# kch3782/torcwa

Measured on AMD Instinct MI355X. Metric: RCWA layer-solves/sec (complex64 I/O) at Fourier order [15,15], higher is better.
Workload: dtype c128 results (mixed-precision eigensolver: fp32 eigendecomposition refined to fp64 by two Newton steps -- fp64 residual and update GEMMs, the correction solved with ONE fp32 LU of the fp32 start; everything else fp64 MFMA); complex64 I/O; 1 GPU; configs[1]: single patterned layer, order=[15,15] (n=1922), 300x300 grid, 128-lambda sweep, glass input half-space; points_total=128, points_per_gpu=128, layer_solves_per_point=1, chunk=128, streams=1, precision=high

## Files before the change

torcwa_amd/csrc/eig.hip:

```cpp
#include "eig.hpp"
#include "prof.hpp"
#include <cstdlib>
#include <string>
#include <vector>

namespace trx {

static inline size_t al256(size_t x) { return (x + 255) & ~(size_t)255; }

static int eig_vec_env() {
    const char* e = getenv("TRX_EIG_VEC");
    const int v = e ? atoi(e) : 0;
    return (v == 0 || v == 1 || v == 3) ? v : 0;
}
static int g_eig_vec = eig_vec_env();
static thread_local int tl_eig_vec = -1, tl_refine = -1;
static thread_local int tl_last_fallback = 0;
static inline int cur_eig_vec() { return tl_eig_vec >= 0 ? tl_eig_vec : g_eig_vec; }
struct EigCallOpts {
    EigCallOpts(unsigned opts) { const int r = opts & 0xF, v = (opts >> 4) & 0xF; tl_refine = r ? r : -1; tl_eig_vec = v ? v : -1; }
    ~EigCallOpts() { tl_refine = -1; tl_eig_vec = -1; }
};
bool eig_uses_mixed(int n, int batch, size_t elem) { return elem == 8 && ((cur_eig_vec() == 3 && n >= 8) || (cur_eig_vec() == 0 && n >= 256 && batch >= 8)); }
int eig_set_knob(const char* key, int value) {
    if (std::string(key) != "eig_vec" || (value != 0 && value != 1 && value != 3)) return TRX_ERR_ARG;
    g_eig_vec = value;
    return TRX_OK;
}


template <class T> size_t eig_ws_bytes_t(int n, int batch);
static size_t eig_ws_bytes_f32(int n, int batch) { return eig_ws_bytes_t<float>(n, batch); }

static size_t mixed_pool_bytes(int n, int batch) {
    const size_t B = batch, N = n;
    return al256(8 * B * N * N) + al256(eig_ws_bytes_f32(n, batch)) + al256(8 * B * N * N) + al256(8 * B * N);
}
static size_t mixed_extra_bytes(int n, int batch) {
    const size_t B = batch, N = n, e = 16;
    const size_t zx = 2 * al256(e * B * N * N), pool = mixed_pool_bytes(n, batch);
    size_t tot = 0;
    if (pool > zx) tot += al256(pool - zx);
    tot += al256(sizeof(int) * B * N) * 3 + al256(sizeof(int) * (B + 2)) * 2 + al256(sizeof(int) * B) + al256(sizeof(int) * 2 * REFINE_EDGE_CAP * B) +
           al256(8 * B) * 2 + al256(8 * 64 * B) + al256(REFINE_CLUSTER_BYTES * B) + al256(e * B * N);
    return tot;
}

template <class T>
size_t eig_ws_bytes_t(int n, int batch) {
    const size_t e = sizeof(cx<T>), B = batch, N = n;
    size_t tot = 0;
    tot += al256(e * B * N * N) * 2;
    tot += al256(e * B * N * EigPlan::HNB) * 2;
    tot += al256(e * B * EigPlan::HNB * EigPlan::HNB);
    tot += al256(e * B * EigPlan::HNB * N) * 2;
    tot += al256(e * B * N * 2 * EigPlan::HNB) * 2;
    tot += al256(e * B * EigPlan::HNB * EigPlan::HNB);
    tot += al256(e * B * N * EigPlan::HGK) * 3 + al256(e * B * EigPlan::HGK * EigPlan::HGK) * 2;
    tot += al256(e * B * EigPlan::HNB) * 2;
    tot += al256(e * B * EigPlan::QW * EigPlan::QW);
    {
        const size_t slots = (size_t)qr_log_slots(n) * qr_chains_for(batch);
        tot += al256(e * B * slots * EigPlan::QW * EigPlan::QW) + al256(sizeof(QrLink) * B * slots);
    }
    tot += al256(e * B * EigPlan::QKC * EigPlan::QNS);
    tot += al256(sizeof(T) * B * N) + al256(sizeof(T) * 3 * B * N) + al256(sizeof(int) * 2 * B);
    tot += al256(sizeof(QrState) * B);
    tot += al256(sizeof(int) * 128 + sizeof(long long) * 24);
    if (eig_uses_mixed(n, batch, sizeof(T))) tot += mixed_extra_bytes(n, batch);
    return tot;
}

template <class T>
void eig_carve(EigBuffers<T>& Bf, void* A, void* ws, int n, int batch) {
    const size_t e = sizeof(cx<T>), B = batch, N = n;
    char* p = (char*)ws;
    auto take = [&](size_t bytes) { char* q = p; p += al256(bytes); return q; };
    Bf.A = (cx<T>*)A;
    Bf.Z = (cx<T>*)take(e * B * N * N);
    Bf.X = (cx<T>*)take(e * B * N * N);
    Bf.mixed_pool = nullptr;
    Bf.mixed_pool_bytes = 0;
    if (eig_uses_mixed(n, batch, sizeof(T))) {
        const size_t zx = 2 * al256(e * B * N * N), pool = mixed_pool_bytes(n, batch);
        if (pool > zx) (void)take(pool - zx);
        Bf.mixed_pool = (char*)Bf.Z;
        Bf.mixed_pool_bytes = pool > zx ? pool : zx;
    }
    Bf.Vp = (cx<T>*)take(e * B * N * EigPlan::HNB);
    Bf.Yp = (cx<T>*)take(e * B * N * EigPlan::HNB);
    Bf.Tp = (cx<T>*)take(e * B * EigPlan::HNB * EigPlan::HNB);
    Bf.W1 = (cx<T>*)take(e * B * EigPlan::HNB * N);
    Bf.W2 = (cx<T>*)take(e * B * EigPlan::HNB * N);
    Bf.YV = (cx<T>*)take(e * B * N * 2 * EigPlan::HNB);
    Bf.BC = (cx<T>*)take(e * B * N * 2 * EigPlan::HNB);
    Bf.Sm = (cx<T>*)take(e * B * EigPlan::HNB * EigPlan::HNB);
    Bf.Vg = (cx<T>*)take(e * B * N * EigPlan::HGK);
    Bf.Wg = (cx<T>*)take(e * B * N * EigPlan::HGK);
    Bf.W2g = (cx<T>*)take(e * B * N * EigPlan::HGK);
    Bf.Tg = (cx<T>*)take(e * B * EigPlan::HGK * EigPlan::HGK);
    Bf.Gg = (cx<T>*)take(e * B * EigPlan::HGK * EigPlan::HGK);
    Bf.tau = (cx<T>*)take(e * B * EigPlan::HNB);
    Bf.tvec = (cx<T>*)take(e * B * EigPlan::HNB);
    Bf.U = (cx<T>*)take(e * B * EigPlan::QW * EigPlan::QW);
    {
        const size_t slots = (size_t)qr_log_slots(n) * qr_chains_for(batch);
        Bf.Ulog = (cx<T>*)take(e * B * slots * EigPlan::QW * EigPlan::QW);
        Bf.links = (QrLink*)take(sizeof(QrLink) * B * slots);
    }
    Bf.shifts = (cx<T>*)take(e * B * EigPlan::QKC * EigPlan::QNS);
    Bf.bal_d = (T*)take(sizeof(T) * B * N);
    Bf.bal_w = (T*)take(sizeof(T) * 3 * B * N);
    Bf.bal_flags = (int*)take(sizeof(int) * 2 * B);
    Bf.st = (QrState*)take(sizeof(QrState) * B);
    Bf.summary = (int*)take(sizeof(int) * 128 + sizeof(long long) * 24);
    Bf.r_piv = Bf.r_linfo = Bf.r_flags = Bf.r_partner = Bf.r_clus = Bf.r_edges = Bf.r_ecount = nullptr;
    Bf.r_eoff = Bf.r_lmax = Bf.r_scan = nullptr;
    Bf.r_tab = nullptr;
    Bf.r_d0 = nullptr;
    if (eig_uses_mixed(n, batch, sizeof(T))) {
        Bf.r_piv = (int*)take(sizeof(int) * B * N);
        Bf.r_partner = (int*)take(sizeof(int) * B * N);
        Bf.r_clus = (int*)take(sizeof(int) * B * N);
        Bf.r_linfo = (int*)take(sizeof(int) * (B + 2));
        Bf.r_flags = (int*)take(sizeof(int) * (B + 2));
        Bf.r_ecount = (int*)take(sizeof(int) * B);
        Bf.r_edges = (int*)take(sizeof(int) * 2 * REFINE_EDGE_CAP * B);
        Bf.r_eoff = (T*)take(8 * B);
        Bf.r_lmax = (T*)take(8 * B);
        Bf.r_scan = (T*)take(8 * 64 * B);
        Bf.r_tab = take(REFINE_CLUSTER_BYTES * B);
        Bf.r_d0 = (cx<T>*)take(e * B * N);
    }
}

namespace {
__global__ __launch_bounds__(256) void cvt_c128_c64_kernel(const cx<double>* __restrict__ in, cx<float>* __restrict__ out, long count) {
    const long i = (long)blockIdx.x * blockDim.x + threadIdx.x;
    if (i < count) { const cx<double> v = in[i]; out[i] = cx<float>((float)v.x, (float)v.y); }
}
int eig_mixed_convert(hipStream_t s, const cx<double>* in, cx<float>* out, long count) {
    TRX_LAUNCH(cvt_c128_c64_kernel, dim3(cdiv_i(count, 256)), dim3(256), 0, s, in, out, count);
    TRX_CHECK_LAUNCH();
    return TRX_OK;
}

template <class T>
__global__ __launch_bounds__(256) void clear_below_subdiag_kernel(cx<T>* __restrict__ Aall, int n) {
    cx<T>* A = Aall + (long)blockIdx.z * n * n;
    const int j = blockIdx.x * blockDim.x + threadIdx.x;
    const int i = blockIdx.y;
    if (j < n && i > j + 1) A[(long)i * n + j] = cx<T>(T(0), T(0));
}

template <class T>
int eig_after_balance(hipStream_t s, const EigBuffers<T>& B, void* w, void* V, int n, int batch, int* info);

template <class T>
__global__ __launch_bounds__(256) void gather_rows_kernel(const T* __restrict__ src, T* __restrict__ dst, const int* __restrict__ idx, long row, int to_compact) {
    const long i = (long)blockIdx.x * blockDim.x + threadIdx.x;
    if (i >= row) return;
    const long j = blockIdx.y, b = idx[j];
    if (to_compact) dst[j * row + i] = src[b * row + i];
    else dst[b * row + i] = src[j * row + i];
}

template <class T>
int eig_redo_subset(hipStream_t s, void* A, void* w, void* V, int n, int batch, int* info, void* ws, size_t ws_bytes, const T* bal_d, const std::vector<int>& bad, int nf) {
    const size_t e = sizeof(cx<T>), N = n, NF = nf;
    struct RouteGuard { int save; RouteGuard() : save(tl_eig_vec) { tl_eig_vec = 1; } ~RouteGuard() { tl_eig_vec = save; } } guard;
    const size_t front = eig_ws_bytes_t<T>(n, nf);
    const size_t tail = al256(e * NF * N * N) * 2 + al256(e * NF * N) + al256(sizeof(T) * NF * N) + al256(sizeof(int) * NF) * 2;
    if (front + tail > ws_bytes) return TRX_ERR_WORKSPACE;
    char* p = (char*)ws + ws_bytes - tail;
    p = (char*)(((size_t)p) & ~(size_t)255);
    if (p < (char*)ws + front) return TRX_ERR_WORKSPACE;
    auto take = [&](size_t bytes) { char* q = p; p += al256(bytes); return q; };
    char* p_save = p;
    p = p_save + al256(e * NF * N * N) * 2;
    cx<T>* wsub = (cx<T>*)take(e * NF * N);
    T* dsub = (T*)take(sizeof(T) * NF * N);
    int* idx = (int*)take(sizeof(int) * NF);
    int* isub = (int*)take(sizeof(int) * NF);
    p = p_save;
    if ((const char*)wsub < (const char*)(bal_d + (size_t)batch * n)) return TRX_ERR_WORKSPACE;
    cx<T>* Asub = (cx<T>*)take(e * NF * N * N);
    cx<T>* Vsub = (cx<T>*)take(e * NF * N * N);
    std::vector<int> hidx;
    for (int b = 0; b < batch; ++b) if (bad[b]) hidx.push_back(b);
    if ((int)hidx.size() != nf) return TRX_ERR_ARG;
    if (hipMemcpyAsync(idx, hidx.data(), sizeof(int) * NF, hipMemcpyHostToDevice, s) != hipSuccess) return TRX_ERR_LAUNCH;
    if (hipStreamSynchronize(s) != hipSuccess) return TRX_ERR_LAUNCH;
    TRX_LAUNCH((gather_rows_kernel<T>), dim3(cdiv_i(n, 256), nf), dim3(256), 0, s, bal_d, dsub, (const int*)idx, (long)n, 1);
    TRX_LAUNCH((gather_rows_kernel<cx<T>>), dim3(cdiv_i((long)n * n, 256), nf), dim3(256), 0, s, (const cx<T>*)A, Asub, (const int*)idx, (long)n * n, 1);
    EigBuffers<T> S;
    eig_carve<T>(S, Asub, ws, n, nf);
    if (hipMemcpyAsync(S.bal_d, dsub, sizeof(T) * NF * N, hipMemcpyDeviceToDevice, s) != hipSuccess) return TRX_ERR_LAUNCH;
    if (hipMemsetAsync(isub, 0, sizeof(int) * NF, s) != hipSuccess) return TRX_ERR_LAUNCH;
    int rc = eig_after_balance<T>(s, S, wsub, Vsub, n, nf, isub);
    if (rc) return rc;
    TRX_LAUNCH((gather_rows_kernel<cx<T>>), dim3(cdiv_i(n, 256), nf), dim3(256), 0, s, (const cx<T>*)wsub, (cx<T>*)w, (const int*)idx, (long)n, 0);
    TRX_LAUNCH((gather_rows_kernel<cx<T>>), dim3(cdiv_i((long)n * n, 256), nf), dim3(256), 0, s, (const cx<T>*)Vsub, (cx<T>*)V, (const int*)idx, (long)n * n, 0);
    TRX_LAUNCH((gather_rows_kernel<int>), dim3(1, nf), dim3(256), 0, s, (const int*)isub, info, (const int*)idx, 1L, 0);
    TRX_CHECK_LAUNCH();
    return TRX_OK;
}

template <class T>
int eig_t(hipStream_t s, void* A, void* w, void* V, int n, int batch, int* info, void* ws, size_t ws_bytes) {
    EigBuffers<T> B;
    eig_carve<T>(B, A, ws, n, batch);
    if (hipMemsetAsync(info, 0, sizeof(int) * batch, s) != hipSuccess) return TRX_ERR_LAUNCH;
    int rc;
    { ProfScope ph(PROF_PH_BALANCE, s, 0, 0);
      rc = balance<T>(s, B, n, batch); }
    if (rc) return rc;
    if constexpr (sizeof(T) == 8) {
        if (eig_uses_mixed(n, batch, sizeof(T))) {
            const size_t Bn = batch, N = n;
            char* p = B.mixed_pool;
            cx<float>* A32 = (cx<float>*)p; p += al256(8 * Bn * N * N);
            void* ws32 = p; p += al256(eig_ws_bytes_f32(n, batch));
            cx<float>* V32 = (cx<float>*)p; p += al256(8 * Bn * N * N);
            cx<float>* w32 = (cx<float>*)p;
            rc = eig_mixed_convert(s, (const cx<double>*)A, A32, (long)Bn * N * N);
            if (rc) return rc;
            rc = eig_t<float>(s, A32, w32, V32, n, batch, B.r_linfo, ws32, eig_ws_bytes_f32(n, batch));
            if (rc) return rc;
            RefineBuffers<T> R;
            R.Rb = B.X; R.LU32 = (cx<float>*)B.Z; R.E32 = R.LU32 + Bn * N * N; R.d0 = B.r_d0; R.piv = B.r_piv; R.linfo = B.r_linfo; R.flags = B.r_flags;
            R.eoff = B.r_eoff; R.lmax = B.r_lmax; R.scan_part = B.r_scan; R.partner = B.r_partner; R.clus = B.r_clus; R.edges = B.r_edges; R.ecount = B.r_ecount; R.tab = B.r_tab;
            int any = 0;
            std::vector<int> bad(batch, 0);
            { ProfScope ph(PROF_PH_REFINE, s, 0, 0);
              rc = eig_refine<T>(s, R, (const cx<T>*)A, V32, w32, (cx<T>*)w, (cx<T>*)V, n, batch, tl_refine > 0 ? tl_refine : refine_steps(), &any, bad.data()); }
            if (rc) return rc;
            tl_last_fallback = any;
            if (!any) return finish_vectors<T>(s, B, n, batch, (cx<T>*)V);
            if (3 * any <= batch) {
                rc = finish_vectors<T>(s, B, n, batch, (cx<T>*)V);
                if (rc) return rc;
                rc = eig_redo_subset<T>(s, A, w, V, n, batch, info, ws, ws_bytes, B.bal_d, bad, any);
                if (rc != TRX_ERR_WORKSPACE) return rc;
            }
            tl_last_fallback = batch;
        }
    }
    return eig_after_balance<T>(s, B, w, V, n, batch, info);
}

template <class T>
int eig_after_balance(hipStream_t s, const EigBuffers<T>& B, void* w, void* V, int n, int batch, int* info) {
    int rc;
    { ProfScope ph(PROF_PH_HESSENBERG, s, 0, 0);
      rc = hessenberg<T>(s, B, n, batch);
      if (rc) return rc;
      TRX_LAUNCH((clear_below_subdiag_kernel<T>), dim3(cdiv_i(n, 256), n, batch), dim3(256), 0, s, B.A, n); }
    { ProfScope ph(PROF_PH_QR, s, 0, 0);
      rc = hessenberg_qr<T>(s, B, n, batch, info); }
    if (rc) return rc;
    ProfScope ph(PROF_PH_VECTORS, s, 0, 0);
    return schur_vectors<T>(s, B, n, batch, (cx<T>*)w, (cx<T>*)V);
}
}

template <class T>
__global__ __launch_bounds__(256) void eigbwd_inner_kernel(const cx<T>* __restrict__ w, const cx<T>* __restrict__ gw, cx<T>* __restrict__ M, int n, T eps) {
    const int b = blockIdx.z, i = blockIdx.y;
    const int j = blockIdx.x * blockDim.x + threadIdx.x;
    if (j >= n) return;
    const cx<T>* wb = w + (long)b * n;
    cx<T>* p = M + ((long)b * n + i) * n + j;
    if (i == j) { *p = gw[(long)b * n + i]; return; }
    const cx<T> sij = wb[j] - wb[i];
    const T den = norm2(sij) + eps;
    *p = cx<T>(sij.x / den, sij.y / den) * (*p);
}
template <class T>
__global__ __launch_bounds__(256) void conj_transpose_kernel(const cx<T>* __restrict__ in, cx<T>* __restrict__ out, int n) {
    __shared__ cx<T> tile[32][33];
    in += (long)blockIdx.z * n * n;
    out += (long)blockIdx.z * n * n;
    const int c0 = blockIdx.x * 32, r0 = blockIdx.y * 32;
    for (int i = threadIdx.y; i < 32; i += 8) {
        const int r = r0 + i, c = c0 + threadIdx.x;
        if (r < n && c < n) tile[i][threadIdx.x] = conj(in[(long)r * n + c]);
    }
    __syncthreads();
    for (int i = threadIdx.y; i < 32; i += 8) {
        const int r = c0 + i, c = r0 + threadIdx.x;
        if (r < n && c < n) out[(long)r * n + c] = tile[threadIdx.x][i];
    }
}
template <class T>
int eig_backward_t(hipStream_t s, const cx<T>* w, const cx<T>* V, const cx<T>* gw, const cx<T>* gV, double eps, int n, int batch, cx<T>* gA,
                   int* piv, int* info, cx<T>* ws) {
    const long nn = (long)n * n;
    const cx<T> one(T(1), T(0)), zero(T(0), T(0));
    cx<T>* M = ws;
    cx<T>* XH = ws + (long)batch * nn;
    int rc = gemm<T>(s, TRX_OP_C, TRX_OP_N, n, n, n, one, V, n, nn, gV, n, nn, zero, M, n, nn, batch); if (rc) return rc;
    TRX_LAUNCH((eigbwd_inner_kernel<T>), dim3(cdiv_i(n, 256), n, batch), dim3(256), 0, s, w, gw, M, n, (T)eps);
    rc = gemm<T>(s, TRX_OP_N, TRX_OP_C, n, n, n, one, M, n, nn, V, n, nn, zero, gA, n, nn, batch); if (rc) return rc;
    TRX_LAUNCH((conj_transpose_kernel<T>), dim3(cdiv_i(n, 32), cdiv_i(n, 32), batch), dim3(32, 8), 0, s, V, XH, n);
    rc = lu_factor<T>(s, XH, n, nn, n, piv, batch, info); if (rc) return rc;
    rc = lu_solve<T>(s, XH, n, nn, n, piv, gA, n, nn, n, batch); if (rc) return rc;
    TRX_CHECK_LAUNCH();
    return TRX_OK;
}

template size_t eig_ws_bytes_t<float>(int, int);
template size_t eig_ws_bytes_t<double>(int, int);
template void eig_carve<float>(EigBuffers<float>&, void*, void*, int, int);
template void eig_carve<double>(EigBuffers<double>&, void*, void*, int, int);

}

using trx::cx;

extern "C" size_t trx_eig_backward_ws_bytes(int dtype, int n, int batch) {
    return (size_t)(dtype == TRX_C128 ? 16 : 8) * 2 * (size_t)batch * n * n;
}

extern "C" int trx_eig_backward(int dtype, const void* w, const void* V, const void* gw, const void* gV, double broadening, int n, int batch,
                                void* gA, int* piv, int* info, void* ws, size_t ws_bytes, void* stream) {
    if (!w || !V || !gw || !gV || !gA || !piv || !info || !ws || n <= 0 || batch <= 0 || !(broadening >= 0.0)) return TRX_ERR_ARG;
    if (ws_bytes < trx_eig_backward_ws_bytes(dtype, n, batch)) return TRX_ERR_WORKSPACE;
    hipStream_t s = trx::api_stream(stream);
    if (dtype == TRX_C64)
        return trx::eig_backward_t<float>(s, (const cx<float>*)w, (const cx<float>*)V, (const cx<float>*)gw, (const cx<float>*)gV, broadening, n, batch,
                                     (cx<float>*)gA, piv, info, (cx<float>*)ws);
    if (dtype == TRX_C128)
        return trx::eig_backward_t<double>(s, (const cx<double>*)w, (const cx<double>*)V, (const cx<double>*)gw, (const cx<double>*)gV, broadening, n, batch,
                                      (cx<double>*)gA, piv, info, (cx<double>*)ws);
    return TRX_ERR_DTYPE;
}

extern "C" int trx_tuning(const char* key, int value) {
    if (!key) return TRX_ERR_ARG;
    int rc = trx::qr_set_knob(key, value);
    if (rc != TRX_OK) rc = trx::lu_set_knob(key, value);
    if (rc != TRX_OK) rc = trx::eig_set_knob(key, value);
    if (rc != TRX_OK) rc = trx::hess_set_knob(key, value);
    if (rc != TRX_OK) rc = trx::gemm_set_knob(key, value);
    if (rc != TRX_OK) rc = trx::refine_set_knob(key, value);
    return rc;
}

extern "C" size_t trx_eig_ws_bytes(int dtype, int n, int batch) {
    if (n <= 0 || batch <= 0) return 0;
    return dtype == TRX_C128 ? trx::eig_ws_bytes_t<double>(n, batch) : trx::eig_ws_bytes_t<float>(n, batch);
}

extern "C" int trx_eig_last_fallback(void) { return trx::tl_last_fallback; }

static inline bool eig_opts_valid(unsigned opts) {
    const unsigned r = opts & 0xF, v = (opts >> 4) & 0xF;
    return r <= 4 && (v == 0 || v == 1 || v == 3) && !(opts >> 8);
}

extern "C" size_t trx_eig_ws_bytes_opts(int dtype, int n, int batch, unsigned opts) {
    if (!eig_opts_valid(opts)) return 0;
    trx::EigCallOpts guard(opts);
    return trx_eig_ws_bytes(dtype, n, batch);
}

extern "C" int trx_eig_opts(int dtype, void* A, void* w, void* V, int n, int batch, int* info, void* ws, size_t ws_bytes, void* stream, unsigned opts) {
    if (!eig_opts_valid(opts)) return TRX_ERR_ARG;
    trx::EigCallOpts guard(opts);
    return trx_eig(dtype, A, w, V, n, batch, info, ws, ws_bytes, stream);
}

extern "C" int trx_eig(int dtype, void* A, void* w, void* V, int n, int batch, int* info, void* ws, size_t ws_bytes,
                       void* stream) {
    if (!A || !w || !V || !info || !ws || n <= 0 || batch <= 0) return TRX_ERR_ARG;
    if (dtype != TRX_C64 && dtype != TRX_C128) return TRX_ERR_DTYPE;
    if (ws_bytes < trx_eig_ws_bytes(dtype, n, batch)) return TRX_ERR_WORKSPACE;
    hipStream_t s = trx::api_stream(stream);
    trx::tl_last_fallback = 0;
    return dtype == TRX_C128 ? trx::eig_t<double>(s, A, w, V, n, batch, info, ws, ws_bytes) : trx::eig_t<float>(s, A, w, V, n, batch, info, ws, ws_bytes);
}
```

torcwa_amd/csrc/eig.hpp:

```cpp
#pragma once
#include "common.hpp"

namespace trx {

struct EigPlan {
    static constexpr int HNB = 32;
    static constexpr int HG = 4;
    static constexpr int HGK = HG * HNB;
    static constexpr int QW = 64;
    static constexpr int QNS = 16;
    static constexpr int QKC = 3;
    static constexpr int QNMIN = 64;
    static constexpr int QAED = 64;
    static constexpr int VNB = 32;
};

struct QrState {
    int ilo, ihi;
    int nch;
    int k[EigPlan::QKC];
    int tau[EigPlan::QKC][2];
    int tau_last[EigPlan::QKC];
    int mode;
    int stall, sweeps;
    int w0[EigPlan::QKC], w1[EigPlan::QKC];
    int fail;
};
enum { QR_CHASE = 0, QR_SMALL_PENDING = 1, QR_SMALL_APPLIED = 2, QR_IDLE = 3, QR_DONE = 4, QR_AED_CHASE = 5 };
struct QrLink { int w0, w1, kind, e; };
enum { QRL_NONE = 0, QRL_CHASE = 1, QRL_DENSE = 2 };
int qr_chains_for(int batch);
int qr_log_slots(int n);

template <class T>
struct EigBuffers {
    cx<T>* A;
    cx<T>* Z;
    cx<T>* X;
    cx<T>* Vp;
    cx<T>* Yp;
    cx<T>* Tp;
    cx<T>* W1;
    cx<T>* W2;
    cx<T>* YV;
    cx<T>* BC;
    cx<T>* Sm;
    cx<T>* Vg;
    cx<T>* Wg;
    cx<T>* W2g;
    cx<T>* Tg;
    cx<T>* Gg;
    cx<T>* tau;
    cx<T>* tvec;
    cx<T>* U;
    cx<T>* Ulog;
    QrLink* links;
    cx<T>* shifts;
    T* bal_d;
    T* bal_w;
    int* bal_flags;
    QrState* st;
    int* summary;
    char* mixed_pool;
    size_t mixed_pool_bytes;
    int *r_piv, *r_linfo, *r_flags, *r_partner, *r_clus, *r_edges, *r_ecount;
    T *r_eoff, *r_lmax, *r_scan;
    void* r_tab;
    cx<T>* r_d0;
};

template <class T>
struct RefineBuffers {
    cx<T>* Rb;
    cx<float>* LU32;
    cx<float>* E32;
    cx<T>* d0;
    int* piv;
    int* linfo;
    int* flags;
    T* eoff;
    T* lmax;
    T* scan_part;
    int* partner;
    int* clus;
    int* edges;
    int* ecount;
    void* tab;
};
constexpr size_t REFINE_CLUSTER_BYTES = 1728 * 1024;
constexpr int REFINE_EDGE_CAP = 16384;
template <class T> int eig_refine(hipStream_t s, const RefineBuffers<T>& R, const cx<T>* A, const cx<float>* V32, const cx<float>* w32, cx<T>* w, cx<T>* V,
                                  int n, int batch, int steps, int* host_any, int* host_bad);
int refine_set_knob(const char* key, int value);
int refine_steps();

template <class T> size_t eig_ws_bytes_t(int n, int batch);
template <class T> void eig_carve(EigBuffers<T>& B, void* A, void* ws, int n, int batch);

template <class T> int balance(hipStream_t s, const EigBuffers<T>& B, int n, int batch);
template <class T> int hessenberg(hipStream_t s, const EigBuffers<T>& B, int n, int batch);
template <class T> int hessenberg_qr(hipStream_t s, const EigBuffers<T>& B, int n, int batch, int* info);
int qr_set_knob(const char* key, int value);
int eig_set_knob(const char* key, int value);
int hess_set_knob(const char* key, int value);
template <class T> int schur_vectors(hipStream_t s, const EigBuffers<T>& B, int n, int batch, cx<T>* w, cx<T>* V);
template <class T> int finish_vectors(hipStream_t s, const EigBuffers<T>& B, int n, int batch, cx<T>* V);

}
```

torcwa_amd/csrc/eig_hess.hip:

```cpp
#include "eig.hpp"
#include <cstdlib>
#include <string>
#include "prof.hpp"

namespace trx {
namespace {

constexpr int HNB = EigPlan::HNB;
constexpr int HCT = 512;
constexpr int HRG = HCT / HNB;

template <class T>
__global__ __launch_bounds__(HCT) void hess_col_kernel(cx<T>* __restrict__ Aall, int n, int p0, int c, int nwg,
                                                        cx<T>* __restrict__ Vall, cx<T>* __restrict__ Tall, cx<T>* __restrict__ tau_all,
                                                        cx<T>* __restrict__ tvec_all, const cx<T>* __restrict__ Bcol_all, const cx<T>* __restrict__ wpart_all) {
    TRX_DYN_SMEM(smem);
    cx<T>* bcol = reinterpret_cast<cx<T>*>(smem);
    cx<T>* part = bcol + n;
    cx<T>* vec = part + HRG * HNB;
    T* red = reinterpret_cast<T*>(vec + HNB);
    const int b = blockIdx.x;
    cx<T>* A = Aall + (long)b * n * n;
    cx<T>* V = Vall + (long)b * n * HNB;
    cx<T>* Tm = Tall + (long)b * HNB * HNB;
    cx<T>* tau = tau_all + (long)b * HNB;
    cx<T>* tvec = tvec_all + (long)b * HNB;
    const cx<T>* Bcol = Bcol_all + (long)b * n;
    const cx<T>* wpart = wpart_all + (long)b * nwg * HNB;
    const int t = threadIdx.x;
    const int cc = t & (HNB - 1), rg = t / HNB;
    const int r0 = p0 + 1, nr = n - r0, j = p0 + c;
    if (c > 0) {
        cx<T> acc(T(0), T(0));
        if (cc < c)
            for (int g = rg; g < nwg; g += HRG) acc += wpart[(long)g * HNB + cc];
        part[rg * HNB + cc] = acc;
        __syncthreads();
        if (t < HNB) {
            cx<T> sraw(T(0), T(0));
            for (int g = 0; g < HRG; ++g) sraw += part[g * HNB + t];
            vec[t] = (t < c) ? sraw : cx<T>(T(0), T(0));
        }
        __syncthreads();
        cx<T> wq(T(0), T(0));
        if (t < c)
            for (int p = 0; p <= t; ++p) cfma_conj(wq, Tm[p * HNB + t], vec[p]);
        __syncthreads();
        if (t < HNB) vec[t] = wq;
        __syncthreads();
    }
    for (int i = t; i < nr; i += blockDim.x) {
        cx<T> v = (c > 0) ? Bcol[r0 + i] : A[(long)(r0 + i) * n + j];
        for (int q = 0; q < c; ++q) cfma(v, -V[(long)(r0 + i) * HNB + q], vec[q]);
        bcol[i] = v;
    }
    __syncthreads();
    const int x0 = j + 1 - r0;
    T ss = T(0);
    for (int i = x0 + 1 + t; i < nr; i += blockDim.x) ss += norm2(bcol[i]);
    ss = wave_sum(ss);
    if ((t & 63) == 0) red[t >> 6] = ss;
    {
        cx<T> acc(T(0), T(0));
        if (cc < c)
            for (int i = x0 + 1 + rg; i < nr; i += HRG) cfma_conj(acc, V[(long)(r0 + i) * HNB + cc], bcol[i]);
        part[rg * HNB + cc] = acc;
    }
    __syncthreads();
    T xn2 = T(0);
    for (int w = 0; w < (int)(blockDim.x >> 6); ++w) xn2 += red[w];
    const cx<T> alpha = bcol[x0];
    cx<T> tau_c, scale;
    T beta;
    const bool vanishing = !(norm2(alpha) + xn2 >= eps_of<T>::safmin / eps_of<T>::value);
    if (vanishing || (xn2 == T(0) && alpha.y == T(0))) {
        tau_c = cx<T>(T(0), T(0));
        scale = cx<T>(T(0), T(0));
        beta = vanishing ? T(0) : alpha.x;
    } else {
        const T nrm = sqrt(norm2(alpha) + xn2);
        beta = (alpha.x >= T(0)) ? -nrm : nrm;
        tau_c = cx<T>((beta - alpha.x) / beta, -alpha.y / beta);
        scale = crecip(cx<T>(alpha.x - beta, alpha.y));
    }
    if (t < HNB) {
        cx<T> u(T(0), T(0));
        for (int g = 0; g < HRG; ++g) u += part[g * HNB + t];
        cx<T> tq(T(0), T(0));
        if (t < c) tq = conj(V[(long)(j + 1) * HNB + t]) + scale * u;
        vec[t] = tq;
        tvec[t] = tq;
    }
    if (t == 0) tau[c] = tau_c;
    __syncthreads();
    if (t < HNB) {
        cx<T> sT(T(0), T(0));
        if (t < c) {
            for (int q = t; q < c; ++q) cfma(sT, Tm[t * HNB + q], vec[q]);
            sT = -(tau_c * sT);
        } else if (t == c) {
            sT = tau_c;
        }
        if (t <= c) Tm[t * HNB + c] = sT;
    }
    for (int i = t; i < nr; i += blockDim.x) {
        const int r = r0 + i;
        cx<T> a, v;
        if (r <= j) { a = bcol[i]; v = cx<T>(T(0), T(0)); }
        else if (r == j + 1) { a = cx<T>(beta, T(0)); v = cx<T>(T(1), T(0)); }
        else { a = cx<T>(T(0), T(0)); v = bcol[i] * scale; }
        A[(long)r * n + j] = a;
        V[(long)r * HNB + c] = v;
    }
    for (int r = t; r < r0; r += blockDim.x) V[(long)r * HNB + c] = cx<T>(T(0), T(0));
}

template <class T, int RPW>
__global__ __launch_bounds__(512) void hess_gemv_kernel(const cx<T>* __restrict__ Aall, int n, int r0, int j, int c, int next,
                                                         const cx<T>* __restrict__ Vall, cx<T>* __restrict__ Yall, const cx<T>* __restrict__ tau_all,
                                                         const cx<T>* __restrict__ tvec_all, cx<T>* __restrict__ Bcol_all, cx<T>* __restrict__ wpart_all,
                                                         int rows_per_block) {
    TRX_DYN_SMEM(smem);
    static_assert(RPW % 2 == 0 && HNB == 32, "two rows per half-wave round");
    cx<T>* v = reinterpret_cast<cx<T>*>(smem);
    cx<T>* wred = v + (n - j - 1) + 2;
    const int b = blockIdx.y;
    const cx<T>* A = Aall + (long)b * n * n;
    const cx<T>* V = Vall + (long)b * n * HNB;
    cx<T>* Y = Yall + (long)b * n * HNB;
    const int len = n - j - 1;
    const bool pairs = sizeof(T) == 4 && (n & 1) == 0;
    const int off = pairs ? ((j + 1) & 1) : 0;
    for (int i = threadIdx.x; i < len; i += blockDim.x) v[i + off] = V[(long)(j + 1 + i) * HNB + c];
    __syncthreads();
    const int lane = threadIdx.x & 63, wid = threadIdx.x >> 6, nw = blockDim.x >> 6;
    const int q = lane & 31, half = lane >> 5;
    const int rbeg = r0 + blockIdx.x * rows_per_block;
    const cx<T> tau_c = tau_all[(long)b * HNB + c];
    const cx<T> tq = (q < c) ? tvec_all[(long)b * HNB + q] : cx<T>(T(0), T(0));
    const cx<T> vjn = (next && q <= c) ? conj(V[(long)(j + 1) * HNB + q]) : cx<T>(T(0), T(0));
    cx<T> wacc(T(0), T(0));
    for (int rr = RPW * wid; rr < rows_per_block; rr += RPW * nw) {
        const int ra = rbeg + rr;
        if (ra >= n) break;
        const cx<T>* row[RPW];
        cx<T> acc[RPW];
#pragma unroll
        for (int k = 0; k < RPW; ++k) {
            const bool ok = (rr + k < rows_per_block) && (ra + k < n);
            row[k] = A + (long)(ok ? ra + k : ra) * n + j + 1;
            acc[k] = cx<T>(T(0), T(0));
        }
        cx<T> yq_[RPW / 2], vq_[RPW / 2], an_[RPW / 2];
#pragma unroll
        for (int kp = 0; kp < RPW / 2; ++kp) {
            const int k = 2 * kp + half, r = ra + k;
            const bool ok = (rr + k < rows_per_block) && (r < n);
            yq_[kp] = (ok && q < c) ? Y[(long)r * HNB + q] : cx<T>(T(0), T(0));
            vq_[kp] = (ok && next && q <= c) ? V[(long)r * HNB + q] : cx<T>(T(0), T(0));
            an_[kp] = (ok && next) ? A[(long)r * n + j + 1] : cx<T>(T(0), T(0));
        }
        constexpr int UNR = sizeof(T) == 4 ? 2 : 1;
        int i = lane;
        if (pairs) {
            if constexpr (sizeof(T) == 4) {
                typedef float pair_t __attribute__((ext_vector_type(4)));
                const int npair = (len - off) >> 1;
                const pair_t* vp = reinterpret_cast<const pair_t*>(v + 2 * off);
                int p = lane;
                for (; p + 64 < npair; p += 128) {
                    pair_t a0[RPW], a1[RPW];
#pragma unroll
                    for (int k = 0; k < RPW; ++k) {
                        const pair_t* rp = reinterpret_cast<const pair_t*>(row[k] + off);
                        a0[k] = rp[p]; a1[k] = rp[p + 64];
                    }
                    const pair_t v0 = vp[p], v1 = vp[p + 64];
#pragma unroll
                    for (int k = 0; k < RPW; ++k) {
                        cfma(acc[k], cx<T>(a0[k].x, a0[k].y), cx<T>(v0.x, v0.y)); cfma(acc[k], cx<T>(a0[k].z, a0[k].w), cx<T>(v0.z, v0.w));
                        cfma(acc[k], cx<T>(a1[k].x, a1[k].y), cx<T>(v1.x, v1.y)); cfma(acc[k], cx<T>(a1[k].z, a1[k].w), cx<T>(v1.z, v1.w));
                    }
                }
                for (; p < npair; p += 64) {
                    const pair_t v0 = vp[p];
#pragma unroll
                    for (int k = 0; k < RPW; ++k) {
                        const pair_t a0 = reinterpret_cast<const pair_t*>(row[k] + off)[p];
                        cfma(acc[k], cx<T>(a0.x, a0.y), cx<T>(v0.x, v0.y)); cfma(acc[k], cx<T>(a0.z, a0.w), cx<T>(v0.z, v0.w));
                    }
                }
                if (off && lane == 0) {
#pragma unroll
                    for (int k = 0; k < RPW; ++k) cfma(acc[k], row[k][0], v[off]);
                }
                if (((len - off) & 1) && lane == 1) {
#pragma unroll
                    for (int k = 0; k < RPW; ++k) cfma(acc[k], row[k][len - 1], v[len - 1 + off]);
                }
            }
            i = len;
        }
        for (; i + 64 * (UNR - 1) < len; i += 64 * UNR) {
            cx<T> a[UNR][RPW], vi[UNR];
#pragma unroll
            for (int u = 0; u < UNR; ++u)
#pragma unroll
                for (int k = 0; k < RPW; ++k) a[u][k] = row[k][i + 64 * u];
#pragma unroll
            for (int u = 0; u < UNR; ++u) vi[u] = v[i + 64 * u + off];
#pragma unroll
            for (int u = 0; u < UNR; ++u)
#pragma unroll
                for (int k = 0; k < RPW; ++k) cfma(acc[k], a[u][k], vi[u]);
        }
        for (; i < len; i += 64) {
            const cx<T> vi = v[i + off];
#pragma unroll
            for (int k = 0; k < RPW; ++k) cfma(acc[k], row[k][i], vi);
        }
#pragma unroll
        for (int k = 0; k < RPW; ++k) { acc[k].x = wave_sum(acc[k].x); acc[k].y = wave_sum(acc[k].y); }
#pragma unroll
        for (int kp = 0; kp < RPW / 2; ++kp) {
            const int k = 2 * kp + half;
            const int r = ra + k;
            const bool ok = (rr + k < rows_per_block) && (r < n);
            const cx<T> yraw = half ? acc[2 * kp + 1] : acc[2 * kp];
            const cx<T> yq = yq_[kp];
            cx<T> corr = yq * tq;
#pragma unroll
            for (int o = 16; o > 0; o >>= 1) { corr.x += __shfl_xor(corr.x, o); corr.y += __shfl_xor(corr.y, o); }
            const cx<T> yfin = tau_c * (yraw - corr);
            if (ok && q == 0) Y[(long)r * HNB + c] = yfin;
            if (next) {
                cx<T> term = (q < c ? yq : (q == c ? yfin : cx<T>(T(0), T(0)))) * vjn;
#pragma unroll
                for (int o = 16; o > 0; o >>= 1) { term.x += __shfl_xor(term.x, o); term.y += __shfl_xor(term.y, o); }
                const cx<T> bnew = ok ? an_[kp] - term : cx<T>(T(0), T(0));
                if (ok && q == 0) Bcol_all[(long)b * n + r] = bnew;
                if (ok && q <= c) cfma_conj(wacc, vq_[kp], bnew);
            }
        }
    }
    if (next) {
        wacc.x += __shfl_xor(wacc.x, 32); wacc.y += __shfl_xor(wacc.y, 32);
        if (lane < HNB) wred[wid * HNB + lane] = wacc;
        __syncthreads();
        if (threadIdx.x < HNB) {
            cx<T> sW(T(0), T(0));
            for (int w = 0; w < nw; ++w) sW += wred[w * HNB + threadIdx.x];
            wpart_all[((long)b * gridDim.x + blockIdx.x) * HNB + threadIdx.x] = sW;
        }
    }
}

template <class T>
__global__ __launch_bounds__(256) void pack_yv_kernel(const cx<T>* __restrict__ Yall, const cx<T>* __restrict__ Vall, cx<T>* __restrict__ YVall, int n, int r0) {
    const int b = blockIdx.y;
    const int r = r0 + blockIdx.x * 4 + (threadIdx.x >> 6), c = threadIdx.x & 63;
    if (r >= n) return;
    const cx<T>* src = (c < HNB) ? Yall : Vall;
    YVall[((long)b * n + r) * 2 * HNB + c] = src[((long)b * n + r) * HNB + (c & (HNB - 1))];
}
template <class T>
__global__ __launch_bounds__(256) void conj_transpose_panel_kernel(const cx<T>* __restrict__ Vall, cx<T>* __restrict__ BCall, int n, int row0, int mt) {
    const int b = blockIdx.z, c = blockIdx.y;
    const int j = blockIdx.x * blockDim.x + threadIdx.x;
    if (j >= mt) return;
    BCall[(long)b * 2 * HNB * n + (long)c * n + j] = conj(Vall[((long)b * n + row0 + j) * HNB + c]);
}


template <class T>
__global__ __launch_bounds__(256) void pack_group_kernel(const cx<T>* __restrict__ Vall, const cx<T>* __restrict__ Tall, cx<T>* __restrict__ Vg_all,
                                                         cx<T>* __restrict__ Tg_all, int n, int g_r0, int r0, int ib, int gp) {
    constexpr int GK = EigPlan::HGK;
    const int b = blockIdx.y;
    const int r = g_r0 + blockIdx.x * 8 + (threadIdx.x >> 5), c = threadIdx.x & 31;
    if (r < n) Vg_all[((long)b * n + r) * GK + gp * HNB + c] = (r >= r0 && c < ib) ? Vall[((long)b * n + r) * HNB + c] : cx<T>(T(0), T(0));
    if (blockIdx.x == 0) {
        cx<T>* Tg = Tg_all + (long)b * GK * GK;
        const cx<T>* Tm = Tall + (long)b * HNB * HNB;
        for (int i = threadIdx.x >> 5; i < HNB; i += 8) {
            for (int q = 0; q < EigPlan::HG; ++q)
                Tg[(long)(gp * HNB + i) * GK + q * HNB + c] = (q == gp && i < ib && c < ib) ? Tm[i * HNB + c] : cx<T>(T(0), T(0));
        }
    }
}

template <class T>
__global__ __launch_bounds__(256) void set_identity_batched(cx<T>* __restrict__ X, int n) {
    cx<T>* M = X + (long)blockIdx.z * n * n;
    const int j = blockIdx.x * blockDim.x + threadIdx.x;
    const int i = blockIdx.y;
    if (j < n) M[(long)i * n + j] = cx<T>(i == j ? T(1) : T(0), T(0));
}

}

static int hess_rpw(int batch) {
    static const int v = [] { const char* e = getenv("TRX_HESS_RPW"); const int x = e ? atoi(e) : 0; return (x == 2 || x == 4) ? x : 0; }();
    return v ? v : (batch >= 64 ? 2 : 4);
}

static int hess_group_env() { const char* e = getenv("TRX_HESS_GROUP"); const int v = e ? atoi(e) : 0; return (v >= 0 && v <= EigPlan::HG) ? v : 0; }
static int g_hess_group = hess_group_env();
int hess_set_knob(const char* key, int value) {
    if (std::string(key) != "hess_group" || value < 0 || value > EigPlan::HG) return TRX_ERR_ARG;
    g_hess_group = value;
    return TRX_OK;
}

template <class T>
static int hess_flush_group(hipStream_t s, const EigBuffers<T>& B, int n, int batch, int g_r0, int np) {
    constexpr int GK = EigPlan::HGK;
    const cx<T> one(T(1), T(0)), mone(T(-1), T(0)), zero(T(0), T(0));
    const long nn = (long)n * n, sVg = (long)n * GK, sTg = (long)GK * GK;
    cx<T>*Vg = B.Vg, *Tg = B.Tg, *Gg = B.Gg, *Wg = B.Wg, *W2g = B.W2g, *A = B.A, *Z = B.Z;
    const int kk = np * HNB, nr = n - g_r0;
    int rc;
    if (np > 1) {
        rc = gemm<T>(s, TRX_OP_C, TRX_OP_N, kk, kk, nr, one, Vg + (long)g_r0 * GK, GK, sVg, Vg + (long)g_r0 * GK, GK, sVg, zero, Gg, GK, sTg, batch); if (rc) return rc;
        auto merge = [&](int a0, int ka, int b0, int kb) {
            int r = gemm<T>(s, TRX_OP_N, TRX_OP_N, ka, kb, kb, one, Gg + (long)a0 * GK + b0, GK, sTg, Tg + (long)b0 * GK + b0, GK, sTg, zero, W2g, GK, sVg, batch);
            if (r) return r;
            return gemm<T>(s, TRX_OP_N, TRX_OP_N, ka, kb, ka, mone, Tg + (long)a0 * GK + a0, GK, sTg, W2g, GK, sVg, zero, Tg + (long)a0 * GK + b0, GK, sTg, batch);
        };
        rc = merge(0, HNB, HNB, HNB); if (rc) return rc;
        if (np == 3) { rc = merge(0, 2 * HNB, 2 * HNB, HNB); if (rc) return rc; }
        if (np == 4) {
            rc = merge(2 * HNB, HNB, 3 * HNB, HNB); if (rc) return rc;
            rc = merge(0, 2 * HNB, 2 * HNB, 2 * HNB); if (rc) return rc;
        }
    }
    if (g_r0 > 0) {
        rc = gemm<T>(s, TRX_OP_N, TRX_OP_N, g_r0, kk, nr, one, A + g_r0, n, nn, Vg + (long)g_r0 * GK, GK, sVg, zero, Wg, GK, sVg, batch); if (rc) return rc;
        rc = gemm<T>(s, TRX_OP_N, TRX_OP_N, g_r0, kk, kk, one, Wg, GK, sVg, Tg, GK, sTg, zero, W2g, GK, sVg, batch); if (rc) return rc;
        rc = gemm<T>(s, TRX_OP_N, TRX_OP_C, g_r0, nr, kk, mone, W2g, GK, sVg, Vg + (long)g_r0 * GK, GK, sVg, one, A + g_r0, n, nn, batch); if (rc) return rc;
    }
    rc = gemm<T>(s, TRX_OP_N, TRX_OP_N, n, kk, nr, one, Z + g_r0, n, nn, Vg + (long)g_r0 * GK, GK, sVg, zero, Wg, GK, sVg, batch); if (rc) return rc;
    rc = gemm<T>(s, TRX_OP_N, TRX_OP_N, n, kk, kk, one, Wg, GK, sVg, Tg, GK, sTg, zero, W2g, GK, sVg, batch); if (rc) return rc;
    rc = gemm<T>(s, TRX_OP_N, TRX_OP_C, n, nr, kk, mone, W2g, GK, sVg, Vg + (long)g_r0 * GK, GK, sVg, one, Z + g_r0, n, nn, batch); if (rc) return rc;
    return TRX_OK;
}

template <class T>
int hessenberg(hipStream_t s, const EigBuffers<T>& B, int n, int batch) {
    const cx<T> one(T(1), T(0)), mone(T(-1), T(0)), zero(T(0), T(0));
    const long nn = (long)n * n, sV = (long)n * HNB, sT = HNB * HNB, sW = (long)HNB * n;
    cx<T>*A = B.A, *Z = B.Z, *V = B.Vp, *Y = B.Yp, *Tm = B.Tp, *W = B.W1, *W2 = B.W2;
    TRX_LAUNCH((set_identity_batched<T>), dim3(cdiv_i(n, 256), n, batch), dim3(256), 0, s, Z, n);
    const size_t sm_col = sizeof(cx<T>) * ((size_t)n + HRG * HNB + HNB) + sizeof(T) * 16;
    const size_t sm_gemv = sizeof(cx<T>) * ((size_t)n + 2 + 8 * HNB);
    if (set_max_dyn_smem((const void*)hess_col_kernel<T>, sm_col) || set_max_dyn_smem((const void*)hess_gemv_kernel<T, 2>, sm_gemv) ||
        set_max_dyn_smem((const void*)hess_gemv_kernel<T, 4>, sm_gemv))
        return TRX_ERR_LAUNCH;
    const int rpw = hess_rpw(batch);
    cx<T>* Bcol = W;
    cx<T>* wpart = W2;
    const int hg = g_hess_group ? g_hess_group : EigPlan::HG;
    int g_r0 = 1, gp = 0;
    for (int p0 = 0; p0 < n - 2; p0 += HNB) {
        const int ib = (n - 2 - p0 < HNB) ? (n - 2 - p0) : HNB;
        const int r0 = p0 + 1, nr = n - r0;
        if (hipMemsetAsync(Tm, 0, sizeof(cx<T>) * sT * batch, s) != hipSuccess) return TRX_ERR_LAUNCH;
        const bool few = (long)cdiv_i(nr, 64) * batch < 256;
        const int rpb = few ? 16 : 64, gthreads = few ? 512 : 256;
        const int nwg = cdiv_i(nr, rpb);
        for (int c = 0; c < ib; ++c) {
            const int j = p0 + c;
            { ProfScope prof(PROF_HESS_COL, s, 0, 0);
              TRX_LAUNCH((hess_col_kernel<T>), dim3(batch), dim3(HCT), sm_col, s, A, n, p0, c, nwg, V, Tm, B.tau, B.tvec, (const cx<T>*)Bcol, (const cx<T>*)wpart); }
            const int next = (c + 1 < ib) ? 1 : 0;
            const size_t smg = sizeof(cx<T>) * ((size_t)(n - j - 1) + 2 + (gthreads / 64) * HNB);
            ProfScope prof(PROF_HESS_GEMV, s, 8.0 * (double)nr * (n - j - 1) * batch, (double)sizeof(cx<T>) * nr * (double)(n - j - 1) * batch);
            if (rpw == 4 && !few)
                TRX_LAUNCH((hess_gemv_kernel<T, 4>), dim3(nwg, batch), dim3(gthreads), smg, s, (const cx<T>*)A, n, r0, j, c, next, (const cx<T>*)V, Y,
                           (const cx<T>*)B.tau, (const cx<T>*)B.tvec, Bcol, wpart, rpb);
            else
                TRX_LAUNCH((hess_gemv_kernel<T, 2>), dim3(nwg, batch), dim3(gthreads), smg, s, (const cx<T>*)A, n, r0, j, c, next, (const cx<T>*)V, Y,
                           (const cx<T>*)B.tau, (const cx<T>*)B.tvec, Bcol, wpart, rpb);
        }
        int rc;
        const int mt = n - p0 - ib;
        if (gp == 0) g_r0 = r0;
        const int t0 = hg > 1 ? g_r0 : 0, tr = r0 - t0;
        if (tr > 0) {
            rc = gemm<T>(s, TRX_OP_N, TRX_OP_N, tr, ib, nr, one, A + (long)t0 * n + r0, n, nn, V + (long)r0 * HNB, HNB, sV, zero, W, HNB, sW, batch); if (rc) return rc;
            rc = gemm<T>(s, TRX_OP_N, TRX_OP_N, tr, ib, ib, one, W, HNB, sW, Tm, HNB, sT, zero, Y + (long)t0 * HNB, HNB, sV, batch); if (rc) return rc;
            rc = gemm<T>(s, TRX_OP_N, TRX_OP_C, tr, nr, ib, mone, Y + (long)t0 * HNB, HNB, sV, V + (long)r0 * HNB, HNB, sV, one, A + (long)t0 * n + r0, n, nn, batch); if (rc) return rc;
        }
        if (mt > 0) {
            cx<T>* At = A + (long)r0 * n + p0 + ib;
            if (ib == HNB) {
                const long sYV = (long)n * 2 * HNB, sBC = (long)2 * HNB * n;
                cx<T>*YV = B.YV, *BC = B.BC, *Sm = B.Sm;
                TRX_LAUNCH((pack_yv_kernel<T>), dim3(cdiv_i(nr, 4), batch), dim3(256), 0, s, (const cx<T>*)Y, (const cx<T>*)V, YV, n, r0);
                TRX_LAUNCH((conj_transpose_panel_kernel<T>), dim3(cdiv_i(mt, 256), HNB, batch), dim3(256), 0, s, (const cx<T>*)V, BC, n, p0 + ib, mt);
                rc = gemm<T>(s, TRX_OP_C, TRX_OP_N, ib, mt, nr, one, V + (long)r0 * HNB, HNB, sV, At, n, nn, zero, W, n, sW, batch); if (rc) return rc;
                rc = gemm<T>(s, TRX_OP_C, TRX_OP_N, ib, ib, nr, one, V + (long)r0 * HNB, HNB, sV, Y + (long)r0 * HNB, HNB, sV, zero, Sm, HNB, sT, batch); if (rc) return rc;
                rc = gemm<T>(s, TRX_OP_N, TRX_OP_N, ib, mt, ib, mone, Sm, HNB, sT, BC, n, sBC, one, W, n, sW, batch); if (rc) return rc;
                rc = gemm<T>(s, TRX_OP_C, TRX_OP_N, ib, mt, ib, one, Tm, HNB, sT, W, n, sW, zero, BC + (long)HNB * n, n, sBC, batch); if (rc) return rc;
                rc = gemm<T>(s, TRX_OP_N, TRX_OP_N, nr, mt, 2 * HNB, mone, YV + (long)r0 * 2 * HNB, 2 * HNB, sYV, BC, n, sBC, one, At, n, nn, batch); if (rc) return rc;
            } else {
                rc = gemm<T>(s, TRX_OP_N, TRX_OP_C, nr, mt, ib, mone, Y + (long)r0 * HNB, HNB, sV, V + (long)(p0 + ib) * HNB, HNB, sV, one, At, n, nn, batch); if (rc) return rc;
                rc = gemm<T>(s, TRX_OP_C, TRX_OP_N, ib, mt, nr, one, V + (long)r0 * HNB, HNB, sV, At, n, nn, zero, W, n, sW, batch); if (rc) return rc;
                rc = gemm<T>(s, TRX_OP_C, TRX_OP_N, ib, mt, ib, one, Tm, HNB, sT, W, n, sW, zero, W2, n, sW, batch); if (rc) return rc;
                rc = gemm<T>(s, TRX_OP_N, TRX_OP_N, nr, mt, ib, mone, V + (long)r0 * HNB, HNB, sV, W2, n, sW, one, At, n, nn, batch); if (rc) return rc;
            }
        }
        if (hg == 1) {
            rc = gemm<T>(s, TRX_OP_N, TRX_OP_N, n, ib, nr, one, Z + r0, n, nn, V + (long)r0 * HNB, HNB, sV, zero, W, HNB, sW, batch); if (rc) return rc;
            rc = gemm<T>(s, TRX_OP_N, TRX_OP_N, n, ib, ib, one, W, HNB, sW, Tm, HNB, sT, zero, W2, HNB, sW, batch); if (rc) return rc;
            rc = gemm<T>(s, TRX_OP_N, TRX_OP_C, n, nr, ib, mone, W2, HNB, sW, V + (long)r0 * HNB, HNB, sV, one, Z + r0, n, nn, batch); if (rc) return rc;
        } else {
            TRX_LAUNCH((pack_group_kernel<T>), dim3(cdiv_i(n - g_r0, 8), batch), dim3(256), 0, s, (const cx<T>*)V, (const cx<T>*)Tm, B.Vg, B.Tg, n, g_r0, r0, ib, gp);
            ++gp;
            if (gp == hg || p0 + HNB >= n - 2) {
                rc = hess_flush_group<T>(s, B, n, batch, g_r0, gp); if (rc) return rc;
                gp = 0;
            }
        }
    }
    TRX_CHECK_LAUNCH();
    return TRX_OK;
}

template int hessenberg<float>(hipStream_t, const EigBuffers<float>&, int, int);
template int hessenberg<double>(hipStream_t, const EigBuffers<double>&, int, int);

}
```

Baseline: 44.11 layer-solves/s.

## Restructure Hessenberg column kernel and stage Householder vector contiguously for GEMV

The Householder column kernel now fuses the column update, the norm reduction and the V^H·b partial products into one strided pass. Each thread keeps several rows in registers, and a cross-lane shuffle sum replaces the separate per-row inner loop over previous reflectors. The kernel also writes the current reflector into a new contiguous per-batch vcur buffer. The GEMV kernel then loads that buffer with vectorized reads instead of gathering a strided column of V. This removes uncoalesced strided loads and an extra sync pass, at the cost of an extra n-length workspace per batch and more register pressure in the column kernel.

```diff
diff --git a/torcwa_amd/csrc/eig.hip b/torcwa_amd/csrc/eig.hip
--- a/torcwa_amd/csrc/eig.hip
+++ b/torcwa_amd/csrc/eig.hip
@@ -58,6 +58,7 @@
     tot += al256(e * B * EigPlan::HNB * EigPlan::HNB);
     tot += al256(e * B * N * EigPlan::HGK) * 3 + al256(e * B * EigPlan::HGK * EigPlan::HGK) * 2;
     tot += al256(e * B * EigPlan::HNB) * 2;
+    tot += al256(e * B * N);
     tot += al256(e * B * EigPlan::QW * EigPlan::QW);
     {
         const size_t slots = (size_t)qr_log_slots(n) * qr_chains_for(batch);
@@ -102,6 +103,7 @@
     Bf.Gg = (cx<T>*)take(e * B * EigPlan::HGK * EigPlan::HGK);
     Bf.tau = (cx<T>*)take(e * B * EigPlan::HNB);
     Bf.tvec = (cx<T>*)take(e * B * EigPlan::HNB);
+    Bf.vcur = (cx<T>*)take(e * B * N);
     Bf.U = (cx<T>*)take(e * B * EigPlan::QW * EigPlan::QW);
     {
         const size_t slots = (size_t)qr_log_slots(n) * qr_chains_for(batch);
diff --git a/torcwa_amd/csrc/eig.hpp b/torcwa_amd/csrc/eig.hpp
--- a/torcwa_amd/csrc/eig.hpp
+++ b/torcwa_amd/csrc/eig.hpp
@@ -52,6 +52,7 @@
     cx<T>* Gg;
     cx<T>* tau;
     cx<T>* tvec;
+    cx<T>* vcur;
     cx<T>* U;
     cx<T>* Ulog;
     QrLink* links;
diff --git a/torcwa_amd/csrc/eig_hess.hip b/torcwa_amd/csrc/eig_hess.hip
--- a/torcwa_amd/csrc/eig_hess.hip
+++ b/torcwa_amd/csrc/eig_hess.hip
@@ -9,11 +9,12 @@
 constexpr int HNB = EigPlan::HNB;
 constexpr int HCT = 512;
 constexpr int HRG = HCT / HNB;
+constexpr int HSW = 8;
 
 template <class T>
 __global__ __launch_bounds__(HCT) void hess_col_kernel(cx<T>* __restrict__ Aall, int n, int p0, int c, int nwg,
                                                         cx<T>* __restrict__ Vall, cx<T>* __restrict__ Tall, cx<T>* __restrict__ tau_all,
-                                                        cx<T>* __restrict__ tvec_all, const cx<T>* __restrict__ Bcol_all, const cx<T>* __restrict__ wpart_all) {
+                                                        cx<T>* __restrict__ tvec_all, cx<T>* __restrict__ vcur_all, const cx<T>* __restrict__ Bcol_all, const cx<T>* __restrict__ wpart_all) {
     TRX_DYN_SMEM(smem);
     cx<T>* bcol = reinterpret_cast<cx<T>*>(smem);
     cx<T>* part = bcol + n;
@@ -25,6 +26,7 @@
     cx<T>* Tm = Tall + (long)b * HNB * HNB;
     cx<T>* tau = tau_all + (long)b * HNB;
     cx<T>* tvec = tvec_all + (long)b * HNB;
+    cx<T>* vcur = vcur_all + (long)b * n;
     const cx<T>* Bcol = Bcol_all + (long)b * n;
     const cx<T>* wpart = wpart_all + (long)b * nwg * HNB;
     const int t = threadIdx.x;
@@ -49,26 +51,39 @@
         if (t < HNB) vec[t] = wq;
         __syncthreads();
     }
-    for (int i = t; i < nr; i += blockDim.x) {
-        cx<T> v = (c > 0) ? Bcol[r0 + i] : A[(long)(r0 + i) * n + j];
-        for (int q = 0; q < c; ++q) cfma(v, -V[(long)(r0 + i) * HNB + q], vec[q]);
-        bcol[i] = v;
-    }
-    __syncthreads();
     const int x0 = j + 1 - r0;
+    const cx<T> zero(T(0), T(0));
+    const cx<T> wq = (cc < c) ? vec[cc] : zero;
+    cx<T> acc = zero;
     T ss = T(0);
-    for (int i = x0 + 1 + t; i < nr; i += blockDim.x) ss += norm2(bcol[i]);
-    ss = wave_sum(ss);
-    if ((t & 63) == 0) red[t >> 6] = ss;
-    {
-        cx<T> acc(T(0), T(0));
-        if (cc < c)
-            for (int i = x0 + 1 + rg; i < nr; i += HRG) cfma_conj(acc, V[(long)(r0 + i) * HNB + cc], bcol[i]);
-        part[rg * HNB + cc] = acc;
-    }
+    for (int below = 0; below < 2; ++below) {
+        const int lo = below ? x0 + 1 : 0, hi = below ? nr : x0 + 1;
+        for (int i0 = lo; i0 < hi; i0 += HRG * HSW) {
+            cx<T> pv[HSW], bb[HSW];
+#pragma unroll
+            for (int u = 0; u < HSW; ++u) {
+                const int i = i0 + u * HRG + rg;
+                const bool ok = i < hi;
+                pv[u] = (ok && cc < c) ? V[(long)(r0 + i) * HNB + cc] : zero;
+                bb[u] = !ok ? zero : (c > 0 ? Bcol[r0 + i] : A[(long)(r0 + i) * n + j]);
+            }
+#pragma unroll
+            for (int u = 0; u < HSW; ++u) {
+                const int i = i0 + u * HRG + rg;
+                cx<T> vw = pv[u] * wq;
+#pragma unroll
+                for (int o = 16; o > 0; o >>= 1) { vw.x += __shfl_xor(vw.x, o); vw.y += __shfl_xor(vw.y, o); }
+                const cx<T> bi = bb[u] - vw;
+                if (cc == 0 && i < hi) bcol[i] = bi;
+                if (below) { cfma_conj(acc, pv[u], bi); ss += norm2(bi); }
+            }
+        }
+    }
+    if (cc == 0) red[rg] = ss;
+    part[rg * HNB + cc] = acc;
     __syncthreads();
     T xn2 = T(0);
-    for (int w = 0; w < (int)(blockDim.x >> 6); ++w) xn2 += red[w];
+    for (int g = 0; g < HRG; ++g) xn2 += red[g];
     const cx<T> alpha = bcol[x0];
     cx<T> tau_c, scale;
     T beta;
@@ -111,14 +126,15 @@
         else { a = cx<T>(T(0), T(0)); v = bcol[i] * scale; }
         A[(long)r * n + j] = a;
         V[(long)r * HNB + c] = v;
-    }
-    for (int r = t; r < r0; r += blockDim.x) V[(long)r * HNB + c] = cx<T>(T(0), T(0));
+        vcur[r] = v;
+    }
+    for (int r = t; r < r0; r += blockDim.x) { V[(long)r * HNB + c] = cx<T>(T(0), T(0)); vcur[r] = cx<T>(T(0), T(0)); }
 }
 
 template <class T, int RPW>
 __global__ __launch_bounds__(512) void hess_gemv_kernel(const cx<T>* __restrict__ Aall, int n, int r0, int j, int c, int next,
                                                          const cx<T>* __restrict__ Vall, cx<T>* __restrict__ Yall, const cx<T>* __restrict__ tau_all,
-                                                         const cx<T>* __restrict__ tvec_all, cx<T>* __restrict__ Bcol_all, cx<T>* __restrict__ wpart_all,
+                                                         const cx<T>* __restrict__ tvec_all, const cx<T>* __restrict__ vcur_all, cx<T>* __restrict__ Bcol_all, cx<T>* __restrict__ wpart_all,
                                                          int rows_per_block) {
     TRX_DYN_SMEM(smem);
     static_assert(RPW % 2 == 0 && HNB == 32, "two rows per half-wave round");
@@ -131,14 +147,27 @@
     const int len = n - j - 1;
     const bool pairs = sizeof(T) == 4 && (n & 1) == 0;
     const int off = pairs ? ((j + 1) & 1) : 0;
-    for (int i = threadIdx.x; i < len; i += blockDim.x) v[i + off] = V[(long)(j + 1 + i) * HNB + c];
-    __syncthreads();
     const int lane = threadIdx.x & 63, wid = threadIdx.x >> 6, nw = blockDim.x >> 6;
     const int q = lane & 31, half = lane >> 5;
     const int rbeg = r0 + blockIdx.x * rows_per_block;
     const cx<T> tau_c = tau_all[(long)b * HNB + c];
     const cx<T> tq = (q < c) ? tvec_all[(long)b * HNB + q] : cx<T>(T(0), T(0));
     const cx<T> vjn = (next && q <= c) ? conj(V[(long)(j + 1) * HNB + q]) : cx<T>(T(0), T(0));
+    const cx<T>* vc = vcur_all + (long)b * n + j + 1;
+    if (pairs) {
+        if constexpr (sizeof(T) == 4) {
+            typedef float pair_t __attribute__((ext_vector_type(4)));
+            const int npair = (len - off) >> 1;
+            const pair_t* src = reinterpret_cast<const pair_t*>(vc + off);
+            pair_t* dst = reinterpret_cast<pair_t*>(v + 2 * off);
+            for (int p = threadIdx.x; p < npair; p += blockDim.x) dst[p] = src[p];
+            if (off && threadIdx.x == 0) v[off] = vc[0];
+            if (((len - off) & 1) && threadIdx.x == 1) v[len - 1 + off] = vc[len - 1];
+        }
+    } else {
+        for (int i = threadIdx.x; i < len; i += blockDim.x) v[i] = vc[i];
+    }
+    __syncthreads();
     cx<T> wacc(T(0), T(0));
     for (int rr = RPW * wid; rr < rows_per_block; rr += RPW * nw) {
         const int ra = rbeg + rr;
@@ -351,7 +380,7 @@
     const long nn = (long)n * n, sV = (long)n * HNB, sT = HNB * HNB, sW = (long)HNB * n;
     cx<T>*A = B.A, *Z = B.Z, *V = B.Vp, *Y = B.Yp, *Tm = B.Tp, *W = B.W1, *W2 = B.W2;
     TRX_LAUNCH((set_identity_batched<T>), dim3(cdiv_i(n, 256), n, batch), dim3(256), 0, s, Z, n);
-    const size_t sm_col = sizeof(cx<T>) * ((size_t)n + HRG * HNB + HNB) + sizeof(T) * 16;
+    const size_t sm_col = sizeof(cx<T>) * ((size_t)n + HRG * HNB + HNB) + sizeof(T) * HRG;
     const size_t sm_gemv = sizeof(cx<T>) * ((size_t)n + 2 + 8 * HNB);
     if (set_max_dyn_smem((const void*)hess_col_kernel<T>, sm_col) || set_max_dyn_smem((const void*)hess_gemv_kernel<T, 2>, sm_gemv) ||
         set_max_dyn_smem((const void*)hess_gemv_kernel<T, 4>, sm_gemv))
@@ -371,16 +400,16 @@
         for (int c = 0; c < ib; ++c) {
             const int j = p0 + c;
             { ProfScope prof(PROF_HESS_COL, s, 0, 0);
-              TRX_LAUNCH((hess_col_kernel<T>), dim3(batch), dim3(HCT), sm_col, s, A, n, p0, c, nwg, V, Tm, B.tau, B.tvec, (const cx<T>*)Bcol, (const cx<T>*)wpart); }
+              TRX_LAUNCH((hess_col_kernel<T>), dim3(batch), dim3(HCT), sm_col, s, A, n, p0, c, nwg, V, Tm, B.tau, B.tvec, B.vcur, (const cx<T>*)Bcol, (const cx<T>*)wpart); }
             const int next = (c + 1 < ib) ? 1 : 0;
             const size_t smg = sizeof(cx<T>) * ((size_t)(n - j - 1) + 2 + (gthreads / 64) * HNB);
             ProfScope prof(PROF_HESS_GEMV, s, 8.0 * (double)nr * (n - j - 1) * batch, (double)sizeof(cx<T>) * nr * (double)(n - j - 1) * batch);
             if (rpw == 4 && !few)
                 TRX_LAUNCH((hess_gemv_kernel<T, 4>), dim3(nwg, batch), dim3(gthreads), smg, s, (const cx<T>*)A, n, r0, j, c, next, (const cx<T>*)V, Y,
-                           (const cx<T>*)B.tau, (const cx<T>*)B.tvec, Bcol, wpart, rpb);
+                           (const cx<T>*)B.tau, (const cx<T>*)B.tvec, (const cx<T>*)B.vcur, Bcol, wpart, rpb);
             else
                 TRX_LAUNCH((hess_gemv_kernel<T, 2>), dim3(nwg, batch), dim3(gthreads), smg, s, (const cx<T>*)A, n, r0, j, c, next, (const cx<T>*)V, Y,
-                           (const cx<T>*)B.tau, (const cx<T>*)B.tvec, Bcol, wpart, rpb);
+                           (const cx<T>*)B.tau, (const cx<T>*)B.tvec, (const cx<T>*)B.vcur, Bcol, wpart, rpb);
         }
         int rc;
         const int mt = n - p0 - ib;
```

Result: no change. 43.94 layer-solves/s (-0.4%).
